# aliabdelkader/FusionTransformer

Measured on AMD Instinct MI355X. Metric: frames/sec fwd+bwd (SemanticKITTI synth), whole job, higher is better.
Workload: dtype f32

## Files before the change

fusiontransformer_amd/_lib.py:

```python
from __future__ import annotations

import ctypes as C
import os

import torch

_HERE = os.path.dirname(os.path.abspath(__file__))
LIB_PATH = os.path.join(_HERE, "csrc", "libftx.so")

_i32, _i64, _f32, _vp, _sz = C.c_int32, C.c_int64, C.c_float, C.c_void_p, C.c_size_t

SIGNATURES = {
    "ftx_version": (C.c_int, []),
    "ftx_last_error": (C.c_char_p, []),
    "ftx_stream_scratch_bytes": (_sz, []),
    "ftx_stream_scratch_attach": (C.c_int, [_vp, _vp, _sz]),
    "ftx_stream_scratch_reset": (C.c_int, [_vp]),
    "ftx_stream_scratch_release": (C.c_int, [_vp]),
    "ftx_hash": (C.c_int, [_vp, _i64, _vp, _vp]),
    "ftx_hash_kernel": (C.c_int, [_vp, _i64, _vp, _i32, _vp, _vp]),
    "ftx_floor_coords": (C.c_int, [_vp, _i64, _i32, _vp, _vp]),
    "ftx_hashtable_capacity": (_i64, [_i64]),
    "ftx_hashtable_build": (C.c_int, [_vp, _i64, _vp, _vp, _i64, _vp]),
    "ftx_hashtable_query": (C.c_int, [_vp, _i64, _vp, _vp, _i64, _vp, _vp]),
# ... 37 lines not shown
    "ftx_spconv_ostat": (C.c_int, [_vp, _i64, _vp, _i64, _vp, _i32, _i32, _i32, _i32, _i32, _vp, _vp, _i32, _vp]),
    "ftx_rows_gemm": (C.c_int, [_vp, _i64, _vp, _i32, _vp, _i32, _i32, _vp, _vp]),
    "ftx_spconv_gemm_block_cols": (_i32, [_i32, _i64, _i32]),
    "ftx_spconv_reduce": (C.c_int, [_vp, _vp, _i64, _i32, _i32, _vp, _vp]),
    "ftx_spconv_reduce_bn_eval": (C.c_int, [_vp, _vp, _i64, _i32, _i32, _vp, _vp, _vp, _vp, _vp, _f32, _i32, _vp, _vp]),
    "ftx_spconv_reduce_stats_blocks": (_i32, [_i64, _i32]),
    "ftx_spconv_reduce_stats": (C.c_int, [_vp, _vp, _i64, _i32, _i32, _vp, _vp, _i32, _vp]),
    "ftx_bn_train_fwd_totals": (C.c_int, [_vp, _vp, _vp, _vp, _vp, _vp, _f32, _f32, _i64, _i32, _i32, _vp, _vp, _vp, _vp, _vp]),
    "ftx_spconv_pairs_wgrad_workspace_bytes": (_sz, [_i64, _i32, _i32, _i32]),
    "ftx_spconv_pairs_wgrad": (C.c_int, [_vp, _i64, _vp, _vp, _i64, _vp, _vp, _i64, _i32, _i32, _i32, _vp, _vp, _sz, _vp]),
    "ftx_spconv_wgrad_resident_blocks": (_i32, [_i32, _i32]),
    "ftx_spconv_wgrad_table_blocks": (_i32, [_i32, _i32, _i32, _i32]),
    "ftx_spconv_pairs_gemm_bf16": (C.c_int, [_vp, _i64, _vp, _vp, _i32, _vp, _i64, _i32, _i32, _i32, _vp, _vp]),
    "ftx_spconv_pairs_gemm_scatter_bf16": (C.c_int, [_vp, _i64, _vp, _vp, _vp, _i32, _vp, _i64, _i32, _i32, _i32, _vp, _i64, _vp]),
    "ftx_rows_gemm_bf16": (C.c_int, [_vp, _i64, _vp, _i32, _vp, _i32, _i32, _vp, _vp]),
    "ftx_spconv_pairs_wgrad_bf16_workspace_bytes": (_sz, [_i64, _i32, _i32, _i32]),
    "ftx_spconv_pairs_wgrad_bf16": (C.c_int, [_vp, _i64, _vp, _vp, _i64, _vp, _vp, _i64, _i32, _i32, _i32, _vp, _vp, _sz, _vp]),
    "ftx_spconv_gemm_bf16_block_cols": (_i32, [_i32, _i64, _i32]),
    "ftx_spconv_wgrad_bf16_table_blocks": (_i32, [_i32, _i32, _i32, _i32]),
    "ftx_bn_workspace_bytes": (_sz, [_i64, _i32]),
    "ftx_bn_train_fwd": (C.c_int, [_vp, _vp, _vp, _vp, _vp, _vp, _f32, _f32, _i64, _i32, _i32, _vp, _vp, _vp, _vp, _sz, _vp]),
    "ftx_bn_eval_fwd": (C.c_int, [_vp, _vp, _vp, _vp, _vp, _vp, _f32, _i64, _i32, _i32, _vp, _vp]),
    "ftx_adam_chunk_elements": (_i32, []),
    "ftx_adam_tensor_bytes": (_i32, []),
    "ftx_adam_step": (C.c_int, [_vp, _vp, _vp, _i32, C.c_double, C.c_double, _f32, _f32, _vp]),
    "ftx_add_layernorm_fwd": (C.c_int, [_vp, _vp, _vp, _vp, _vp, _f32, _i64, _i32, _vp, _vp, _vp, _vp, _vp]),
    "ftx_layernorm_bwd_workspace_bytes": (_sz, [_i64, _i32]),
    "ftx_add_layernorm_bwd": (C.c_int, [_vp, _vp, _vp, _vp, _vp, _vp, _i64, _i32, _i32, _vp, _vp, _vp, _sz, _vp]),
    "ftx_colsum_workspace_bytes": (_sz, [_i64, _i32]),
    "ftx_colsum": (C.c_int, [_vp, _i64, _i32, _vp, _vp, _sz, _vp]),
    "ftx_attn_fwd": (C.c_int, [_vp, _i32, _i32, _i32, _i32, _f32, _vp, _vp, _vp]),
    "ftx_attn_bwd_workspace_bytes": (_sz, [_i32, _i32, _i32]),
    "ftx_attn_bwd": (C.c_int, [_vp, _vp, _vp, _vp, _i32, _i32, _i32, _i32, _f32, _vp, _vp, _sz, _vp]),
    "ftx_attn_fwd_tiled": (C.c_int, [_vp, _i32, _i32, _i32, _i32, _f32, _vp, _vp, _i32, _i32, _vp]),
    "ftx_attn_bwd_tiled": (C.c_int, [_vp, _vp, _vp, _vp, _i32, _i32, _i32, _i32, _f32, _vp, _vp, _sz, _i32, _i32, _vp]),
    "ftx_attn_fwd_bf16": (C.c_int, [_vp, _i32, _i32, _i32, _i32, _f32, _vp, _vp, _i32, _i32, _vp]),
    "ftx_attn_bwd_bf16": (C.c_int, [_vp, _vp, _vp, _vp, _i32, _i32, _i32, _i32, _f32, _vp, _vp, _sz, _i32, _i32, _vp]),
    "ftx_dense_gemm_bf16": (C.c_int, [_vp, _vp, _i32, _vp, _vp, _i64, _i32, _i32, _i32, _vp, _vp, _vp]),
    "ftx_dense_wgrad_bf16_workspace_bytes": (_sz, [_i64, _i32, _i32]),
    "ftx_dense_wgrad_bf16": (C.c_int, [_vp, _vp, _i64, _i32, _i32, _vp, _vp, _sz, _vp]),
    "ftx_dense_bf16_tile": (C.c_int, [_i32, _i64, _i32, _i32, _vp, _vp, _vp]),
    "ftx_dense_gemm_split": (C.c_int, [_vp, _vp, _i32, _vp, _vp, _i64, _i32, _i32, _i32, _vp, _vp, _vp]),
    "ftx_dense_wgrad_split_workspace_bytes": (_sz, [_i64, _i32, _i32]),
    "ftx_dense_wgrad_split": (C.c_int, [_vp, _vp, _i64, _i32, _i32, _vp, _vp, _sz, _vp]),
    "ftx_dense_split_tile": (C.c_int, [_i32, _i64, _i32, _i32, _vp, _vp, _vp]),
    "ftx_fusion_loss_workspace_bytes": (_sz, []),
    "ftx_fusion_loss": (C.c_int, [_vp, _vp, _vp, _vp, _vp, _vp, _f32, _i64, _i32, _i32, _vp, _vp, _vp, _vp, _vp, _vp, _vp, _vp, _sz, _vp]),
    "ftx_fusion_loss_mix": (C.c_int, [_vp, _vp, _vp, _vp, _vp, _vp, _f32, _f32, _i64, _i32, _i32, _vp, _vp, _vp, _vp, _vp, _vp, _vp, _vp, _sz, _vp]),
    "ftx_seg_loss_workspace_bytes": (_sz, []),
    "ftx_seg_loss": (C.c_int, [_vp, _vp, _vp, _i64, _i32, _i32, _vp, _vp, _vp, _vp, _sz, _vp]),
    "ftx_project_points": (C.c_int, [_vp, _i64, _vp, _i32, _i32, _vp, _vp, _vp]),
    "ftx_eval_scatter_back": (C.c_int, [_vp, _vp, _i64, _i32, _vp, _vp, _i64, _vp, _vp, _vp, _vp, _vp, _vp, _vp, _vp, _vp]),
    "ftx_bn_train_bwd": (C.c_int, [_vp, _vp, _vp, _vp, _vp, _vp, _vp, _i64, _i32, _i32, _vp, _vp, _vp, _vp, _vp, _sz, _vp]),
    "ftx_color_jitter_workspace_bytes": (_sz, [_i32, _i32]),
    "ftx_color_jitter_u8": (C.c_int, [_vp, _i64, _i32, _i32, _i32, _vp, _vp, _i32, _vp, _vp, _sz, _vp]),
    "ftx_color_jitter_chw": (C.c_int, [_vp, _i64, _i32, _i32, _i32, _vp, _vp, _i32, _i32, _vp, _vp, _vp, _vp, _sz, _vp]),
    "ftx_resize_ksize": (_i32, [_i32, _i32]),
    "ftx_resize_coeffs_host": (C.c_int, [_i32, _i32, _vp, _vp]),
    "ftx_resize_workspace_bytes": (_sz, [_i32, _i32, _i32, _i32, _i32]),
    "ftx_resize_bilinear_u8": (C.c_int, [_vp, _i64, _i64, _i32, _i32, _i32, _i32, _vp, _vp, _i32, _vp, _vp, _i32, _i32, _i32, _vp, _vp, _sz, _vp]),
    "ftx_rows_concat": (C.c_int, [_vp, _i32, _vp, _i32, _i64, _vp, _vp]),
    "ftx_rows_add": (C.c_int, [_vp, _vp, _i64, _i32, _vp, _vp]),
    "ftx_spvcnn_layer_bytes": (_i32, []),
    "ftx_spvcnn_op_bytes": (_i32, []),
    "ftx_spvcnn_map_bytes": (_i32, []),
    "ftx_spvcnn_pv_bytes": (_i32, []),
# ... 64 lines not shown
```

fusiontransformer_amd/csrc/ftx_attn.hip:

```cpp
#include "ftx_common.h"
#include "ftx_mfma.h"

using namespace ftx;

constexpr int HD = 64;
constexpr int TS = 68;
constexpr float LOG2E = 1.4426950408889634f;
constexpr float LN2 = 0.6931471805599453f;

__device__ inline int acc_row(int g, int h) { return (g & 3) + 8 * (g >> 2) + 4 * h; }

__device__ inline float exp2_raw(float x) { return __builtin_amdgcn_exp2f(x); }

__device__ inline const float *qkv_row(const float *qkv, int b, int t, int which, int hd, int T, int nh) {
  return qkv + ((((int64_t)b * T + t) * 3 + which) * nh + hd) * HD;
}

__device__ inline void load_frag(const float *row, int h, bool valid, float (&f)[32]) {
#pragma unroll
  for (int t = 0; t < 8; ++t) {
    float4 v = make_float4(0.f, 0.f, 0.f, 0.f);
    if (valid) v = *(const float4 *)(row + 8 * t + 4 * h);
    f[4 * t + 0] = v.x; f[4 * t + 1] = v.y; f[4 * t + 2] = v.z; f[4 * t + 3] = v.w;
  }
// ... 209 lines not shown
    const float inv = 1.f / l;
    float *op = out + (((int64_t)b * T + q) * nh + hd) * HD;
#pragma unroll
    for (int g4 = 0; g4 < 4; ++g4) {
      int r = acc_row(4 * g4, h);
      *(float4 *)(op + r) = make_float4(o0[4 * g4] * inv, o0[4 * g4 + 1] * inv, o0[4 * g4 + 2] * inv, o0[4 * g4 + 3] * inv);
      *(float4 *)(op + 32 + r) = make_float4(o1[4 * g4] * inv, o1[4 * g4 + 1] * inv, o1[4 * g4 + 2] * inv, o1[4 * g4 + 3] * inv);
    }
    if (h == 0) lse[((int64_t)b * nh + hd) * T + q] = (m + log2f(l)) * LN2;
  }
}

__global__ void attn_delta_kernel(const float *__restrict__ o, const float *__restrict__ go, int64_t rows, int T, int nh, float *__restrict__ delta) {
  const int64_t gid = (blockIdx.x * (int64_t)blockDim.x + threadIdx.x) >> 4;
  const int sub = threadIdx.x & 15;
  if (gid >= rows) return;
  float4 a = *(const float4 *)(o + gid * HD + sub * 4);
  float4 g = *(const float4 *)(go + gid * HD + sub * 4);
  float s = a.x * g.x + a.y * g.y + a.z * g.z + a.w * g.w;
#pragma unroll
  for (int off = 8; off > 0; off >>= 1) s += __shfl_xor(s, off, 16);
  if (sub == 0) {
    int64_t bt = gid / nh;
    int hd = (int)(gid - bt * nh);
    int64_t bb = bt / T;
    int t = (int)(bt - bb * T);
    delta[(bb * nh + hd) * T + t] = s;
  }
}

template <int QW, int SPLIT>
__global__ __launch_bounds__(64 * QW * SPLIT) void attn_bwd_kv_kernel(const float *__restrict__ qkv, const float *__restrict__ go,
                                                                      const float *__restrict__ lse, const float *__restrict__ delta, int T,
                                                                      int nh, float scale, float *__restrict__ gqkv) {
  constexpr int NT = 64 * QW;
  __shared__ __attribute__((aligned(16))) float smem[smem_floats<QW, SPLIT, 64, 64>()];
  const int tid = threadIdx.x % NT, grp = threadIdx.x / NT;
  float *Qs = smem + grp * (2 * 32 * TS + 64), *Gs = Qs + 32 * TS, *s_lse = Gs + 32 * TS, *s_delta = s_lse + 32;
  const int wave = tid >> 6, lane = tid & 63, l31 = lane & 31, h = lane >> 5;
  const int hd = blockIdx.y, b = blockIdx.z;
  const int key = blockIdx.x * (32 * QW) + wave * 32 + l31;
  const bool kv = key < T;
  const bool wave_live = blockIdx.x * (32 * QW) + wave * 32 < T;
  const float sl2 = scale * LOG2E;

  float kf[32], vf[32];
  load_frag(qkv_row(qkv, b, kv ? key : 0, 1, hd, T, nh), h, kv, kf);
  load_frag(qkv_row(qkv, b, kv ? key : 0, 2, hd, T, nh), h, kv, vf);
#pragma unroll
  for (int i = 0; i < 32; ++i) kf[i] *= sl2;

  f32x16 acc[4];
#pragma unroll
  for (int t = 0; t < 4; ++t)
#pragma unroll
    for (int g = 0; g < 16; ++g) acc[t][g] = 0.f;

  const int ntiles = (T + 31) / 32;
  const int iters = (ntiles + SPLIT - 1) / SPLIT;
  float4 rq[512 / NT], rg[512 / NT];
  tile_prefetch<NT>(qkv, b, hd, 0, grp * 32, T, nh, tid, rq);
  tile_prefetch_o<NT>(go, b, hd, grp * 32, T, nh, tid, rg);
  for (int it = 0; it < iters; ++it) {
    const int qt = it * SPLIT + grp;
    tile_store<NT>(Qs, tid, rq);
    tile_store<NT>(Gs, tid, rg);
    if (tid < 32) {
      int t = qt * 32 + tid;
      s_lse[tid] = t < T ? lse[((int64_t)b * nh + hd) * T + t] * LOG2E : 0.f;
      s_delta[tid] = t < T ? delta[((int64_t)b * nh + hd) * T + t] : 0.f;
    }
    group_sync<QW>();
    if (it + 1 < iters) {
      tile_prefetch<NT>(qkv, b, hd, 0, (qt + SPLIT) * 32, T, nh, tid, rq);
      tile_prefetch_o<NT>(go, b, hd, (qt + SPLIT) * 32, T, nh, tid, rg);
    }
    if (qt < ntiles && wave_live) {
      f32x16 s, dp;
#pragma unroll
      for (int g = 0; g < 16; ++g) s[g] = dp[g] = 0.f;
      mfma_lds_x_frag(Qs, l31, h, kf, s);
      mfma_lds_x_frag(Gs, l31, h, vf, dp);
#pragma unroll
      for (int g = 0; g < 16; ++g) {
        const int r = acc_row(g, h);
        const float p = exp2_raw(s[g] - s_lse[r]);
        s[g] = p;
        dp[g] = p * (dp[g] - s_delta[r]) * scale;
      }
      if (qt == ntiles - 1) {
#pragma unroll
        for (int g = 0; g < 16; ++g)
          if (qt * 32 + acc_row(g, h) >= T) s[g] = dp[g] = 0.f;
      }
      mfma_ldsT_x_acc(Gs, 0, l31, h, s, acc[0]);
      mfma_ldsT_x_acc(Gs, 32, l31, h, s, acc[1]);
      mfma_ldsT_x_acc(Qs, 0, l31, h, dp, acc[2]);
      mfma_ldsT_x_acc(Qs, 32, l31, h, dp, acc[3]);
    }
    group_sync<QW>();
  }
  merge_sum<QW, SPLIT, 4>(smem, grp, wave, lane, acc);
  if (kv && grp == 0) {
    float *kp = gqkv + ((((int64_t)b * T + key) * 3 + 1) * nh + hd) * HD;
    float *vp = gqkv + ((((int64_t)b * T + key) * 3 + 2) * nh + hd) * HD;
#pragma unroll
    for (int g4 = 0; g4 < 4; ++g4) {
      int r = acc_row(4 * g4, h);
      *(float4 *)(vp + r) = make_float4(acc[0][4 * g4], acc[0][4 * g4 + 1], acc[0][4 * g4 + 2], acc[0][4 * g4 + 3]);
      *(float4 *)(vp + 32 + r) = make_float4(acc[1][4 * g4], acc[1][4 * g4 + 1], acc[1][4 * g4 + 2], acc[1][4 * g4 + 3]);
      *(float4 *)(kp + r) = make_float4(acc[2][4 * g4], acc[2][4 * g4 + 1], acc[2][4 * g4 + 2], acc[2][4 * g4 + 3]);
      *(float4 *)(kp + 32 + r) = make_float4(acc[3][4 * g4], acc[3][4 * g4 + 1], acc[3][4 * g4 + 2], acc[3][4 * g4 + 3]);
    }
  }
}

template <int QW, int SPLIT>
__global__ __launch_bounds__(64 * QW * SPLIT) void attn_bwd_q_kernel(const float *__restrict__ qkv, const float *__restrict__ go,
                                                                     const float *__restrict__ lse, const float *__restrict__ delta, int T,
                                                                     int nh, float scale, float *__restrict__ gqkv) {
  constexpr int NT = 64 * QW;
  __shared__ __attribute__((aligned(16))) float smem[smem_floats<QW, SPLIT, 32, 0>()];
  const int tid = threadIdx.x % NT, grp = threadIdx.x / NT;
  float *Ks = smem + grp * (2 * 32 * TS), *Vs = Ks + 32 * TS;
  const int wave = tid >> 6, lane = tid & 63, l31 = lane & 31, h = lane >> 5;
  const int hd = blockIdx.y, b = blockIdx.z;
// ... 31 lines not shown
    if (kt < ntiles && wave_live) {
      f32x16 st, dpt;
#pragma unroll
      for (int g = 0; g < 16; ++g) st[g] = dpt[g] = 0.f;
      mfma_lds_x_frag(Ks, l31, h, qf, st);
      mfma_lds_x_frag(Vs, l31, h, gf, dpt);
#pragma unroll
      for (int g = 0; g < 16; ++g) {
        const float p = exp2_raw(st[g] - my_lse);
        dpt[g] = p * (dpt[g] - my_delta) * scale;
      }
      if (kt == ntiles - 1) {
#pragma unroll
        for (int g = 0; g < 16; ++g)
          if (kt * 32 + acc_row(g, h) >= T) dpt[g] = 0.f;
      }
      mfma_ldsT_x_acc(Ks, 0, l31, h, dpt, acc[0]);
      mfma_ldsT_x_acc(Ks, 32, l31, h, dpt, acc[1]);
    }
    group_sync<QW>();
  }
  merge_sum<QW, SPLIT, 2>(smem, grp, wave, lane, acc);
  if (qv && grp == 0) {
    float *qp = gqkv + ((((int64_t)b * T + q) * 3 + 0) * nh + hd) * HD;
#pragma unroll
    for (int g4 = 0; g4 < 4; ++g4) {
      int r = acc_row(4 * g4, h);
      *(float4 *)(qp + r) = make_float4(acc[0][4 * g4], acc[0][4 * g4 + 1], acc[0][4 * g4 + 2], acc[0][4 * g4 + 3]);
      *(float4 *)(qp + 32 + r) = make_float4(acc[1][4 * g4], acc[1][4 * g4 + 1], acc[1][4 * g4 + 2], acc[1][4 * g4 + 3]);
    }
  }
}

static int attn_check(const char *who, int b, int t, int h, int d) {
  FTX_REQUIRE(b >= 1 && t >= 1 && h >= 1, "%s: bad size", who);
  FTX_REQUIRE(d == HD, "%s: head dim must be 64 (got %d)", who, d);
  FTX_REQUIRE(b <= 65535 && h <= 65535, "%s: batch / heads exceed the grid limits", who);
  return FTX_OK;
}

static bool attn_tiling_built(int qw, int split) {
  return (qw == 0 && split == 0) || (qw == 4 && split == 2) || (qw == 2 && (split == 2 || split == 4)) ||
         (qw == 1 && (split == 2 || split == 4 || split == 8));
}
static void attn_config(int b, int t, int h, bool backward, int &qw, int &split) {
  if (qw != 0) return;
  const int64_t wave_tiles = (int64_t)ceil_div(t, 32) * h * b;
  const int64_t simds = 4 * 256;
  if (wave_tiles * 4 <= simds) { qw = 1; split = backward ? 4 : 8; }
  else if (wave_tiles * 2 <= simds) { qw = 2; split = 4; }
  else { qw = 4; split = 2; }
}

#define ATTN_DISPATCH(KERNEL, ...)                                                                               \
  do {                                                                                                           \
    dim3 grid((unsigned)ceil_div(t, 32 * qw), (unsigned)h, (unsigned)b);                                         \
    if (qw == 4) KERNEL<4, 2><<<grid, 512, 0, st>>>(__VA_ARGS__);                                                \
    else if (qw == 2 && split == 2) KERNEL<2, 2><<<grid, 256, 0, st>>>(__VA_ARGS__);                             \
    else if (qw == 2) KERNEL<2, 4><<<grid, 512, 0, st>>>(__VA_ARGS__);                                           \
    else if (split == 2) KERNEL<1, 2><<<grid, 128, 0, st>>>(__VA_ARGS__);                                        \
    else if (split == 4) KERNEL<1, 4><<<grid, 256, 0, st>>>(__VA_ARGS__);                                        \
    else KERNEL<1, 8><<<grid, 512, 0, st>>>(__VA_ARGS__);                                                        \
  } while (0)

extern "C" int ftx_attn_fwd_tiled(const float *qkv, int32_t b, int32_t t, int32_t h, int32_t d, float scale, float *out, float *lse, int32_t qw,
                                  int32_t split, void *stream) {
  int rc = attn_check("ftx_attn_fwd", b, t, h, d);
  if (rc != FTX_OK) return rc;
  FTX_REQUIRE(qkv && out && lse, "ftx_attn_fwd: null pointer");
  FTX_REQUIRE(attn_tiling_built(qw, split), "ftx_attn_fwd_tiled: (%d, %d) is not a built tiling", qw, split);
  hipStream_t st = (hipStream_t)stream;
  attn_config(b, t, h, false, qw, split);
  ATTN_DISPATCH(attn_fwd_kernel, qkv, t, h, scale, out, lse);
  return check_launch("ftx_attn_fwd");
}

extern "C" int ftx_attn_fwd(const float *qkv, int32_t b, int32_t t, int32_t h, int32_t d, float scale, float *out, float *lse, void *stream) {
  return ftx_attn_fwd_tiled(qkv, b, t, h, d, scale, out, lse, 0, 0, stream);
}

extern "C" size_t ftx_attn_bwd_workspace_bytes(int32_t b, int32_t t, int32_t h) {
  if (b <= 0 || t <= 0 || h <= 0) return 256;
  return sizeof(float) * (size_t)b * t * h + 256;
}

extern "C" int ftx_attn_bwd_tiled(const float *qkv, const float *out, const float *grad_out, const float *lse, int32_t b, int32_t t, int32_t h,
                                  int32_t d, float scale, float *grad_qkv, void *workspace, size_t workspace_bytes, int32_t qw, int32_t split,
                                  void *stream) {
  int rc = attn_check("ftx_attn_bwd", b, t, h, d);
  if (rc != FTX_OK) return rc;
  FTX_REQUIRE(qkv && out && grad_out && lse && grad_qkv && workspace, "ftx_attn_bwd: null pointer");
  FTX_REQUIRE(attn_tiling_built(qw, split), "ftx_attn_bwd_tiled: (%d, %d) is not a built tiling", qw, split);
  if (workspace_bytes < ftx_attn_bwd_workspace_bytes(b, t, h)) {
    set_error("ftx_attn_bwd: workspace %zu < required %zu", workspace_bytes, ftx_attn_bwd_workspace_bytes(b, t, h));
    return FTX_EWORKSPACE;
  }
  hipStream_t st = (hipStream_t)stream;
  float *delta = (float *)workspace;
  const int64_t rows = (int64_t)b * t * h;
  attn_delta_kernel<<<(unsigned)ceil_div(rows * 16, 256), 256, 0, st>>>(out, grad_out, rows, t, h, delta);
  attn_config(b, t, h, true, qw, split);
  ATTN_DISPATCH(attn_bwd_kv_kernel, qkv, grad_out, lse, delta, t, h, scale, grad_qkv);
  ATTN_DISPATCH(attn_bwd_q_kernel, qkv, grad_out, lse, delta, t, h, scale, grad_qkv);
  return check_launch("ftx_attn_bwd");
}

extern "C" int ftx_attn_bwd(const float *qkv, const float *out, const float *grad_out, const float *lse, int32_t b, int32_t t, int32_t h,
                            int32_t d, float scale, float *grad_qkv, void *workspace, size_t workspace_bytes, void *stream) {
  return ftx_attn_bwd_tiled(qkv, out, grad_out, lse, b, t, h, d, scale, grad_qkv, workspace, workspace_bytes, 0, 0, stream);
}

constexpr int RS = 72;
constexpr int CS = 36;
constexpr int IMG = 32 * RS;
static_assert(32 * RS == 64 * CS, "row and col images are the same size");

__device__ inline bf16x4 cvt4(float4 v) { return (bf16x4){(__bf16)v.x, (__bf16)v.y, (__bf16)v.z, (__bf16)v.w}; }

__device__ inline void load_frag_bf16(const float *row, int h, bool valid, bf16x8 (&f)[4]) {
#pragma unroll
  for (int s = 0; s < 4; ++s) {
    float4 a = make_float4(0.f, 0.f, 0.f, 0.f), b = a;
    if (valid) {
      a = *(const float4 *)(row + 16 * s + 8 * h);
      b = *(const float4 *)(row + 16 * s + 8 * h + 4);
    }
    f[s] = __builtin_shufflevector(cvt4(a), cvt4(b), 0, 1, 2, 3, 4, 5, 6, 7);
  }
}
__device__ inline bf16x8 rowimg_frag(const __bf16 *img, int row, int s, int h) { return *(const bf16x8 *)(img + row * RS + 16 * s + 8 * h); }
__device__ inline bf16x8 colimg_frag(const __bf16 *img, int row, int s, int h) {
  const __bf16 *p = img + row * CS + 16 * s + 4 * h;
  return __builtin_shufflevector(*(const bf16x4 *)p, *(const bf16x4 *)(p + 8), 0, 1, 2, 3, 4, 5, 6, 7);
}
__device__ inline bf16x8 acc_frag(const f32x16 &x, int s) {
  bf16x8 r;
#pragma unroll
// ... 386 lines not shown
```

fusiontransformer_amd/csrc/ftx_index.hip:

```cpp
#include <cstring>
#include <cstdlib>
#include "ftx_common.h"
#include <rocprim/device/device_radix_sort.hpp>
#include <rocprim/device/device_select.hpp>
#include <string>

namespace ftx {
static thread_local std::string g_err;
void set_error(const char *fmt, ...) {
  char buf[512];
  va_list ap;
  va_start(ap, fmt);
  vsnprintf(buf, sizeof(buf), fmt, ap);
  va_end(ap);
  g_err = buf;
}
}

using namespace ftx;

extern "C" int ftx_version(void) { return 101; }
extern "C" const char *ftx_last_error(void) { return ftx::g_err.c_str(); }

__global__ void hash_kernel(const int4 *__restrict__ coords, int64_t n, int64_t *__restrict__ out) {
  for (int64_t i = blockIdx.x * (int64_t)blockDim.x + threadIdx.x; i < n; i += (int64_t)gridDim.x * blockDim.x) {
    int4 c = coords[i];
    out[i] = fnv_hash4(c.x, c.y, c.z, c.w);
  }
}

extern "C" int ftx_hash(const int32_t *coords, int64_t n, int64_t *out, void *stream) {
  FTX_REQUIRE(n >= 0, "ftx_hash: n < 0");
  if (n == 0) return FTX_OK;
  FTX_REQUIRE(coords && out, "ftx_hash: null pointer");
  hash_kernel<<<grid_for(n, 256), 256, 0, (hipStream_t)stream>>>((const int4 *)coords, n, out);
  return check_launch("ftx_hash");
}

__global__ void hash_kernel_offsets(const int4 *__restrict__ coords, int64_t n, const int32_t *__restrict__ offsets, int k,
                                    int64_t *__restrict__ out) {
  int64_t total = n * k;
  for (int64_t e = blockIdx.x * (int64_t)blockDim.x + threadIdx.x; e < total; e += (int64_t)gridDim.x * blockDim.x) {
    int kk = (int)(e / n);
    int64_t i = e - (int64_t)kk * n;
    int4 c = coords[i];
    out[e] = fnv_hash4(c.x + offsets[kk * 3 + 0], c.y + offsets[kk * 3 + 1], c.z + offsets[kk * 3 + 2], c.w);
  }
}

extern "C" int ftx_hash_kernel(const int32_t *coords, int64_t n, const int32_t *offsets, int32_t k, int64_t *out, void *stream) {
  FTX_REQUIRE(n >= 0 && k >= 0, "ftx_hash_kernel: negative size");
  if (n == 0 || k == 0) return FTX_OK;
  FTX_REQUIRE(coords && offsets && out, "ftx_hash_kernel: null pointer");
  hash_kernel_offsets<<<grid_for(n * k, 256), 256, 0, (hipStream_t)stream>>>((const int4 *)coords, n, offsets, k, out);
// ... 483 lines not shown
```

fusiontransformer_amd/functional.py:

```python
from __future__ import annotations

import ctypes
import functools

import numpy as np
import torch

from . import _lib
from ._lib import check, ptr, req, stream

I32, I64, F32 = torch.int32, torch.int64, torch.float32


def _empty(shape, dtype, like):
    return torch.empty(shape, dtype=dtype, device=like.device)


_SCRATCH = {}
_WS_BYTES = {}


def _ws_bytes(fn_name, *args):
    key = (fn_name,) + args
    v = _WS_BYTES.get(key)
# ... 1052 lines not shown
            g = gs if gs is not None else torch.zeros(ctx.shape, dtype=F32, device=s.device)
            gyb = colsum(g.reshape(-1, g.shape[-1])) if ctx.with_y_bias else None
            return g, g, gyb, None, None, None
        gx, gparams = _ln_backward(gh, gs, s, weight, stats, ctx.with_y_bias)
        gx = gx.view(ctx.shape)
        return gx, gx, (gparams[2] if ctx.with_y_bias else None), gparams[0], gparams[1], None


def layer_norm(x, weight, bias, eps=1e-5):
    return _LayerNorm.apply(x, weight, bias, eps)


def add_layer_norm(x, y, weight, bias, eps=1e-5, y_bias=None):
    return _AddLayerNorm.apply(x, y, y_bias, weight, bias, eps)


def colsum(x: torch.Tensor) -> torch.Tensor:
    L = _lib.load()
    x = req(x.contiguous(), F32, "colsum x", 2)
    rows, cols = x.shape
    out = _empty((cols,), F32, x)
    ws_bytes = _ws_bytes("ftx_colsum_workspace_bytes", rows, cols)
    ws = _scratch(ws_bytes, x)
    check(L.ftx_colsum(ptr(x), rows, cols, ptr(out), ptr(ws), ws_bytes, stream()), "ftx_colsum")
    return out


_ATTENTION = {False: ("ftx_attn_fwd_tiled", "attn_fwd", "ftx_attn_bwd_tiled", "attn_bwd"),
              True: ("ftx_attn_fwd_bf16", "attn_fwd_bf16", "ftx_attn_bwd_bf16", "attn_bwd_bf16")}


class _Attention(torch.autograd.Function):
    @staticmethod
    def forward(ctx, qkv, scale, tiling=(0, 0), bf16=False):
        L = _lib.load()
        fn, kind = _ATTENTION[bf16][:2]
        qkv = req(qkv.contiguous(), F32, "attention qkv", 5)
        b, t, three, h, d = qkv.shape
        if three != 3 or d != 64:
            raise ValueError(f"attention: qkv must be (B, T, 3, heads, 64), got {tuple(qkv.shape)}")
        out = _empty((b, t, h * d), F32, qkv)
        lse = _empty((b, h, t), F32, qkv)
        qw, split = int(tiling[0]), int(tiling[1])
        _log_launch(kind, dict(b=b, t=t, h=h, d=d, products=2), lambda: check(getattr(L, fn)(
            ptr(qkv), b, t, h, d, float(scale), ptr(out), ptr(lse), qw, split, stream()), fn))
        ctx.save_for_backward(qkv, out, lse)
        ctx.scale, ctx.tiling, ctx.bf16 = float(scale), (qw, split), bf16
        return out

    @staticmethod
    def backward(ctx, go):
        L = _lib.load()
        fn, kind = _ATTENTION[ctx.bf16][2:]
        qkv, out, lse = ctx.saved_tensors
        b, t, _, h, d = qkv.shape
        go = req(go.contiguous(), F32, "attention grad", 3)
        gqkv = torch.empty_like(qkv)
        ws_bytes = int(L.ftx_attn_bwd_workspace_bytes(b, t, h))
        ws = torch.empty((ws_bytes,), dtype=torch.uint8, device=qkv.device)
        _log_launch(kind, dict(b=b, t=t, h=h, d=d, products=7), lambda: check(getattr(L, fn)(
            ptr(qkv), ptr(out), ptr(go), ptr(lse), b, t, h, d, ctx.scale, ptr(gqkv), ptr(ws), ws_bytes, ctx.tiling[0], ctx.tiling[1], stream()), fn))
        return gqkv, None, None, None


def attention(qkv, scale, tiling=(0, 0), bf16=False):
    return _Attention.apply(qkv, scale, tiling, bool(bf16))


EPI_NONE, EPI_BIAS, EPI_BIAS_GELU, EPI_DGELU = 0, 1, 2, 3
_DENSE_MODES = ("bf16", "split")


def vit_linear_supported(x, weight):
    n, k = weight.shape
    return (x.is_cuda and weight.is_cuda and x.dtype == F32 and weight.dtype == F32 and x.shape[-1] == k and k % 64 == 0 and n % 64 == 0
            and x.numel() // k <= (1 << 30))


def _dense_gemm(a, w, w_kn, epi, bias=None, pre_in=None, with_pre=False, mode="bf16"):
    L = _lib.load()
    m, kr = a.shape
    n = w.shape[1] if w_kn else w.shape[0]
    out = _empty((m, n), F32, a)
    pre = _empty((m, n), F32, a) if with_pre else None
    _log_launch("vit_gemm_" + mode, dict(m=m, n=n, k=kr, w_kn=w_kn, epi=epi), lambda: check(getattr(L, "ftx_dense_gemm_" + mode)(
        ptr(a), ptr(w), w_kn, ptr(bias), ptr(pre_in), m, n, kr, epi, ptr(out), ptr(pre), stream()), "ftx_dense_gemm_" + mode))
    return out, pre


def _dense_wgrad(g, x, mode="bf16"):
    L = _lib.load()
    m, n = g.shape
    k = x.shape[1]
    dw = _empty((n, k), F32, g)
    ws_bytes = _ws_bytes(f"ftx_dense_wgrad_{mode}_workspace_bytes", m, n, k)
    ws = _scratch(ws_bytes, g)
    _log_launch("vit_wgrad_" + mode, dict(m=m, n=n, k=k), lambda: check(getattr(L, "ftx_dense_wgrad_" + mode)(
        ptr(g), ptr(x), m, n, k, ptr(dw), ptr(ws), ws_bytes, stream()), "ftx_dense_wgrad_" + mode))
    return dw
# ... 381 lines not shown
```

include/ftx.h:

```cpp
#ifndef FTX_H
#define FTX_H

#include <stddef.h>
#include <stdint.h>

#ifdef __cplusplus
extern "C" {
#endif

#define FTX_OK 0
#define FTX_EINVAL -1
#define FTX_ELAUNCH -2
#define FTX_EWORKSPACE -3

int ftx_version(void);
const char *ftx_last_error(void);

size_t ftx_stream_scratch_bytes(void);
int ftx_stream_scratch_attach(void *stream, void *buffer, size_t bytes);
int ftx_stream_scratch_reset(void *stream);
int ftx_stream_scratch_release(void *stream);


int ftx_hash(const int32_t *coords, int64_t n, int64_t *out, void *stream);
// ... 83 lines not shown
int32_t ftx_spconv_wgrad_table_blocks(int32_t mi, int32_t wmg, int32_t ni, int32_t wng);

int ftx_spconv_pairs_gemm_bf16(const float *A, int64_t rows_a, const int32_t *gather, const float *W, int32_t w_transposed, const int32_t *koff, int64_t n_pairs, int32_t ca, int32_t co, int32_t kvol, float *tmp, void *stream);
int ftx_spconv_pairs_gemm_scatter_bf16(const float *A, int64_t rows_a, const int32_t *gather, const int32_t *scatter, const float *W, int32_t w_transposed, const int32_t *koff, int64_t n_pairs, int32_t ca, int32_t co, int32_t kvol, float *out, int64_t rows_out, void *stream);
int ftx_rows_gemm_bf16(const float *A, int64_t n, const float *W, int32_t w_transposed, const float *bias, int32_t ca, int32_t co, float *out, void *stream);
size_t ftx_spconv_pairs_wgrad_bf16_workspace_bytes(int64_t n_pairs, int32_t ca, int32_t cg, int32_t kvol);
int ftx_spconv_pairs_wgrad_bf16(const float *A, int64_t rows_a, const int32_t *idx_a, const float *G, int64_t rows_g, const int32_t *idx_g, const int32_t *koff, int64_t n_pairs, int32_t ca, int32_t cg, int32_t kvol, float *dW, void *workspace, size_t workspace_bytes, void *stream);
int32_t ftx_spconv_gemm_bf16_block_cols(int32_t co, int64_t n_pairs, int32_t kvol);
int32_t ftx_spconv_wgrad_bf16_table_blocks(int32_t mi, int32_t wmg, int32_t ni, int32_t wng);


size_t ftx_bn_workspace_bytes(int64_t n, int32_t c);
int ftx_bn_train_fwd(const float *x, const float *residual, const float *gamma, const float *beta, float *running_mean, float *running_var, float momentum, float eps, int64_t n, int32_t c, int32_t relu, float *y, float *save_mean, float *save_invstd, void *workspace, size_t workspace_bytes, void *stream);
int ftx_bn_train_fwd_totals(const float *x, const float *residual, const float *gamma, const float *beta, float *running_mean, float *running_var, float momentum, float eps, int64_t n, int32_t c, int32_t relu, float *y, float *save_mean, float *save_invstd, const double *totals, void *stream);

int ftx_bn_eval_fwd(const float *x, const float *residual, const float *gamma, const float *beta, const float *running_mean, const float *running_var, float eps, int64_t n, int32_t c, int32_t relu, float *y, void *stream);
int ftx_bn_train_bwd(const float *grad_y, const float *x, const float *y, const float *gamma, const float *beta, const float *save_mean, const float *save_invstd, int64_t n, int32_t c, int32_t relu, float *grad_x, float *grad_residual, float *grad_gamma, float *grad_beta, void *workspace, size_t workspace_bytes, void *stream);

int32_t ftx_adam_chunk_elements(void);
int32_t ftx_adam_tensor_bytes(void);
int ftx_adam_step(const void *table, const int32_t *chunk_tensor, const int64_t *chunk_offset, int32_t n_chunks, double beta1, double beta2, float eps, float weight_decay, void *stream);

int ftx_add_layernorm_fwd(const float *x, const float *y, const float *y_bias, const float *gamma, const float *beta, float eps, int64_t rows, int32_t c, float *s_out, float *h_out, float *mean, float *rstd, void *stream);
size_t ftx_layernorm_bwd_workspace_bytes(int64_t rows, int32_t c);
int ftx_add_layernorm_bwd(const float *grad_h, const float *grad_s, const float *s, const float *gamma, const float *mean, const float *rstd, int64_t rows, int32_t c, int32_t with_y_bias, float *grad_x, float *grad_params, void *workspace, size_t workspace_bytes, void *stream);

size_t ftx_colsum_workspace_bytes(int64_t rows, int32_t cols);
int ftx_colsum(const float *x, int64_t rows, int32_t cols, float *out, void *workspace, size_t workspace_bytes, void *stream);


int ftx_attn_fwd(const float *qkv, int32_t b, int32_t t, int32_t h, int32_t d, float scale, float *out, float *lse, void *stream);
size_t ftx_attn_bwd_workspace_bytes(int32_t b, int32_t t, int32_t h);
int ftx_attn_bwd(const float *qkv, const float *out, const float *grad_out, const float *lse, int32_t b, int32_t t, int32_t h, int32_t d, float scale, float *grad_qkv, void *workspace, size_t workspace_bytes, void *stream);
int ftx_attn_fwd_tiled(const float *qkv, int32_t b, int32_t t, int32_t h, int32_t d, float scale, float *out, float *lse, int32_t qw, int32_t split, void *stream);
int ftx_attn_bwd_tiled(const float *qkv, const float *out, const float *grad_out, const float *lse, int32_t b, int32_t t, int32_t h, int32_t d, float scale, float *grad_qkv, void *workspace, size_t workspace_bytes, int32_t qw, int32_t split, void *stream);
int ftx_attn_fwd_bf16(const float *qkv, int32_t b, int32_t t, int32_t h, int32_t d, float scale, float *out, float *lse, int32_t qw, int32_t split, void *stream);
int ftx_attn_bwd_bf16(const float *qkv, const float *out, const float *grad_out, const float *lse, int32_t b, int32_t t, int32_t h, int32_t d, float scale, float *grad_qkv, void *workspace, size_t workspace_bytes, int32_t qw, int32_t split, void *stream);

#define FTX_EPI_NONE 0
#define FTX_EPI_BIAS 1
#define FTX_EPI_BIAS_GELU 2
#define FTX_EPI_DGELU 3
int ftx_dense_gemm_bf16(const float *A, const float *W, int32_t w_kn, const float *bias, const float *pre_in, int64_t m, int32_t n, int32_t k, int32_t epilogue, float *out, float *pre_out, void *stream);
size_t ftx_dense_wgrad_bf16_workspace_bytes(int64_t m, int32_t n, int32_t k);
int ftx_dense_wgrad_bf16(const float *dY, const float *X, int64_t m, int32_t n, int32_t k, float *dW, void *workspace, size_t workspace_bytes, void *stream);
int ftx_dense_bf16_tile(int32_t form, int64_t m, int32_t n, int32_t k, int32_t *tile_m_host, int32_t *tile_n_host, int32_t *split_host);

int ftx_dense_gemm_split(const float *A, const float *W, int32_t w_kn, const float *bias, const float *pre_in, int64_t m, int32_t n, int32_t k, int32_t epilogue, float *out, float *pre_out, void *stream);
size_t ftx_dense_wgrad_split_workspace_bytes(int64_t m, int32_t n, int32_t k);
int ftx_dense_wgrad_split(const float *dY, const float *X, int64_t m, int32_t n, int32_t k, float *dW, void *workspace, size_t workspace_bytes, void *stream);
int ftx_dense_split_tile(int32_t form, int64_t m, int32_t n, int32_t k, int32_t *tile_m_host, int32_t *tile_n_host, int32_t *split_host);

size_t ftx_fusion_loss_workspace_bytes(void);
int ftx_fusion_loss_mix(const float *lidar_logit, const float *img_logit, const float *lidar_logit2, const float *img_logit2, const int64_t *label, const float *class_weights, float ce_scale, float lambda_xm, int64_t n, int32_t c, int32_t ignore_index, float *losses, float *grad_lidar, float *grad_img, float *grad_lidar2, float *grad_img2, int64_t *conf3d, int64_t *conf2d, void *workspace, size_t workspace_bytes, void *stream);
int ftx_fusion_loss(const float *lidar_logit, const float *img_logit, const float *lidar_logit2, const float *img_logit2, const int64_t *label, const float *class_weights, float lambda_xm, int64_t n, int32_t c, int32_t ignore_index, float *losses, float *grad_lidar, float *grad_img, float *grad_lidar2, float *grad_img2, int64_t *conf3d, int64_t *conf2d, void *workspace, size_t workspace_bytes, void *stream);

size_t ftx_seg_loss_workspace_bytes(void);
int ftx_seg_loss(const float *logit, const int64_t *label, const float *class_weights, int64_t n, int32_t c, int32_t ignore_index, float *loss, float *grad, int64_t *conf, void *workspace, size_t workspace_bytes, void *stream);

int ftx_eval_scatter_back(const float *logits3d, const float *logits2d, int64_t n_rows, int32_t num_classes, const int64_t *inverse, const int32_t *gt, int64_t m, const int32_t *class_labels, int32_t *pred3d, int32_t *pred2d, int32_t *pred_ens, int64_t *conf3d, int64_t *conf2d, int64_t *conf_ens, int32_t *bad_flag, void *stream);

int ftx_project_points(const float *points, int64_t n, const float *proj_matrix, int32_t width, int32_t height, uint8_t *keep, float *rowcol, void *stream);

#define FTX_JITTER_BRIGHTNESS 0
#define FTX_JITTER_CONTRAST 1
#define FTX_JITTER_SATURATION 2
// ... 57 lines not shown
```

Before: 149.3.

## Hand off dS from KV backward kernel to Q backward instead of recomputing

The KV backward kernel now writes the score gradient dS tile to a workspace buffer. A new Q-gradient kernel reads dS and K and multiplies them, so it no longer recomputes QK^T, the exponentials and dO·V^T. The hand-off path is chosen automatically when the dS buffer fits in 256 MB. This trades recompute FLOPs for an extra T×T-sized global write and read plus a larger workspace.

```diff
diff --git a/fusiontransformer_amd/_lib.py b/fusiontransformer_amd/_lib.py
--- a/fusiontransformer_amd/_lib.py
+++ b/fusiontransformer_amd/_lib.py
@@ -93,6 +93,8 @@
     "ftx_attn_fwd": (C.c_int, [_vp, _i32, _i32, _i32, _i32, _f32, _vp, _vp, _vp]),
     "ftx_attn_bwd_workspace_bytes": (_sz, [_i32, _i32, _i32]),
     "ftx_attn_bwd": (C.c_int, [_vp, _vp, _vp, _vp, _i32, _i32, _i32, _i32, _f32, _vp, _vp, _sz, _vp]),
+    "ftx_attn_bwd_mode_workspace_bytes": (_sz, [_i32, _i32, _i32, _i32]),
+    "ftx_attn_bwd_mode": (C.c_int, [_vp, _vp, _vp, _vp, _i32, _i32, _i32, _i32, _f32, _vp, _vp, _sz, _i32, _i32, _i32, _vp]),
     "ftx_attn_fwd_tiled": (C.c_int, [_vp, _i32, _i32, _i32, _i32, _f32, _vp, _vp, _i32, _i32, _vp]),
     "ftx_attn_bwd_tiled": (C.c_int, [_vp, _vp, _vp, _vp, _i32, _i32, _i32, _i32, _f32, _vp, _vp, _sz, _i32, _i32, _vp]),
     "ftx_attn_fwd_bf16": (C.c_int, [_vp, _i32, _i32, _i32, _i32, _f32, _vp, _vp, _i32, _i32, _vp]),
diff --git a/fusiontransformer_amd/csrc/ftx_attn.hip b/fusiontransformer_amd/csrc/ftx_attn.hip
--- a/fusiontransformer_amd/csrc/ftx_attn.hip
+++ b/fusiontransformer_amd/csrc/ftx_attn.hip
@@ -265,7 +265,7 @@
 template <int QW, int SPLIT>
 __global__ __launch_bounds__(64 * QW * SPLIT) void attn_bwd_kv_kernel(const float *__restrict__ qkv, const float *__restrict__ go,
                                                                       const float *__restrict__ lse, const float *__restrict__ delta, int T,
-                                                                      int nh, float scale, float *__restrict__ gqkv) {
+                                                                      int nh, float scale, float *__restrict__ gqkv, float *__restrict__ ds) {
   constexpr int NT = 64 * QW;
   __shared__ __attribute__((aligned(16))) float smem[smem_floats<QW, SPLIT, 64, 64>()];
   const int tid = threadIdx.x % NT, grp = threadIdx.x / NT;
@@ -325,6 +325,19 @@
 #pragma unroll
         for (int g = 0; g < 16; ++g)
           if (qt * 32 + acc_row(g, h) >= T) s[g] = dp[g] = 0.f;
+      }
+      if (ds) {
+        const int TP = 32 * ntiles;
+        float *tile = ds + (((int64_t)b * nh + hd) * T + __builtin_amdgcn_readfirstlane(qt) * 32) * TP;
+        const unsigned lane_off = 4 * h * TP + key;
+        if (qt == ntiles - 1) {
+#pragma unroll
+          for (int g = 0; g < 16; ++g)
+            if (qt * 32 + acc_row(g, h) < T) (tile + acc_row(g, 0) * TP)[lane_off] = kv ? dp[g] : 0.f;
+        } else {
+#pragma unroll
+          for (int g = 0; g < 16; ++g) (tile + acc_row(g, 0) * TP)[lane_off] = kv ? dp[g] : 0.f;
+        }
       }
       mfma_ldsT_x_acc(Gs, 0, l31, h, s, acc[0]);
       mfma_ldsT_x_acc(Gs, 32, l31, h, s, acc[1]);
@@ -422,6 +435,68 @@
   }
 }
 
+__device__ inline void ds_prefetch(const float *dsrow, int kt, bool valid, float4 (&r)[4]) {
+#pragma unroll
+  for (int j = 0; j < 4; ++j) {
+    float4 v = make_float4(0.f, 0.f, 0.f, 0.f);
+    if (valid) v = *(const float4 *)(dsrow + kt * 32 + 8 * j);
+    r[j] = v;
+  }
+}
+template <int QW, int SPLIT>
+__global__ __launch_bounds__(64 * QW * SPLIT) void attn_bwd_q_handoff_kernel(const float *__restrict__ qkv, const float *__restrict__ ds, int T,
+                                                                             int nh, float *__restrict__ gqkv) {
+  constexpr int NT = 64 * QW;
+  __shared__ __attribute__((aligned(16))) float smem[cmax(SPLIT * 32 * TS, cmax(SPLIT / 2, 1) * QW * 32 * 64)];
+  const int tid = threadIdx.x % NT, grp = threadIdx.x / NT;
+  float *Ks = smem + grp * (32 * TS);
+  const int wave = tid >> 6, lane = tid & 63, l31 = lane & 31, h = lane >> 5;
+  const int hd = blockIdx.y, b = blockIdx.z;
+  const int q = blockIdx.x * (32 * QW) + wave * 32 + l31;
+  const bool qv = q < T;
+  const bool wave_live = blockIdx.x * (32 * QW) + wave * 32 < T;
+
+  f32x16 acc[2];
+#pragma unroll
+  for (int g = 0; g < 16; ++g) acc[0][g] = acc[1][g] = 0.f;
+
+  const int ntiles = (T + 31) / 32;
+  const int iters = (ntiles + SPLIT - 1) / SPLIT;
+  const float *dsrow = ds + (((int64_t)b * nh + hd) * T + (qv ? q : 0)) * (32 * ntiles) + 4 * h;
+  float4 rk[512 / NT], rd[4];
+  tile_prefetch<NT>(qkv, b, hd, 1, grp * 32, T, nh, tid, rk);
+  ds_prefetch(dsrow, grp, qv && grp < ntiles, rd);
+  for (int it = 0; it < iters; ++it) {
+    const int kt = it * SPLIT + grp;
+    tile_store<NT>(Ks, tid, rk);
+    f32x16 dst;
+#pragma unroll
+    for (int j = 0; j < 4; ++j) {
+      dst[4 * j + 0] = rd[j].x; dst[4 * j + 1] = rd[j].y; dst[4 * j + 2] = rd[j].z; dst[4 * j + 3] = rd[j].w;
+    }
+    group_sync<QW>();
+    if (it + 1 < iters) {
+      tile_prefetch<NT>(qkv, b, hd, 1, (kt + SPLIT) * 32, T, nh, tid, rk);
+      ds_prefetch(dsrow, kt + SPLIT, qv && kt + SPLIT < ntiles, rd);
+    }
+    if (kt < ntiles && wave_live) {
+      mfma_ldsT_x_acc(Ks, 0, l31, h, dst, acc[0]);
+      mfma_ldsT_x_acc(Ks, 32, l31, h, dst, acc[1]);
+    }
+    group_sync<QW>();
+  }
+  merge_sum<QW, SPLIT, 2>(smem, grp, wave, lane, acc);
+  if (qv && grp == 0) {
+    float *qp = gqkv + ((((int64_t)b * T + q) * 3 + 0) * nh + hd) * HD;
+#pragma unroll
+    for (int g4 = 0; g4 < 4; ++g4) {
+      int r = acc_row(4 * g4, h);
+      *(float4 *)(qp + r) = make_float4(acc[0][4 * g4], acc[0][4 * g4 + 1], acc[0][4 * g4 + 2], acc[0][4 * g4 + 3]);
+      *(float4 *)(qp + 32 + r) = make_float4(acc[1][4 * g4], acc[1][4 * g4 + 1], acc[1][4 * g4 + 2], acc[1][4 * g4 + 3]);
+    }
+  }
+}
+
 static int attn_check(const char *who, int b, int t, int h, int d) {
   FTX_REQUIRE(b >= 1 && t >= 1 && h >= 1, "%s: bad size", who);
   FTX_REQUIRE(d == HD, "%s: head dim must be 64 (got %d)", who, d);
@@ -469,30 +544,53 @@
   return ftx_attn_fwd_tiled(qkv, b, t, h, d, scale, out, lse, 0, 0, stream);
 }
 
+constexpr size_t ATTN_HANDOFF_CAP = (size_t)256 << 20;
+static size_t attn_delta_bytes(int b, int t, int h) { return (sizeof(float) * (size_t)b * t * h + 255) / 256 * 256; }
+static size_t attn_ds_bytes(int b, int t, int h) { return sizeof(float) * (size_t)b * h * t * (32 * (size_t)ceil_div(t, 32)); }
+static int attn_bwd_rule(int b, int t, int h) { return attn_ds_bytes(b, t, h) <= ATTN_HANDOFF_CAP ? 1 : 0; }
+
+extern "C" size_t ftx_attn_bwd_mode_workspace_bytes(int32_t b, int32_t t, int32_t h, int32_t mode) {
+  if (b <= 0 || t <= 0 || h <= 0) return 256;
+  if (mode != 1) return sizeof(float) * (size_t)b * t * h + 256;
+  return attn_delta_bytes(b, t, h) + attn_ds_bytes(b, t, h);
+}
+
 extern "C" size_t ftx_attn_bwd_workspace_bytes(int32_t b, int32_t t, int32_t h) {
   if (b <= 0 || t <= 0 || h <= 0) return 256;
-  return sizeof(float) * (size_t)b * t * h + 256;
-}
-
-extern "C" int ftx_attn_bwd_tiled(const float *qkv, const float *out, const float *grad_out, const float *lse, int32_t b, int32_t t, int32_t h,
-                                  int32_t d, float scale, float *grad_qkv, void *workspace, size_t workspace_bytes, int32_t qw, int32_t split,
-                                  void *stream) {
+  return ftx_attn_bwd_mode_workspace_bytes(b, t, h, attn_bwd_rule(b, t, h));
+}
+
+extern "C" int ftx_attn_bwd_mode(const float *qkv, const float *out, const float *grad_out, const float *lse, int32_t b, int32_t t, int32_t h,
+                                 int32_t d, float scale, float *grad_qkv, void *workspace, size_t workspace_bytes, int32_t qw, int32_t split,
+                                 int32_t mode, void *stream) {
   int rc = attn_check("ftx_attn_bwd", b, t, h, d);
   if (rc != FTX_OK) return rc;
   FTX_REQUIRE(qkv && out && grad_out && lse && grad_qkv && workspace, "ftx_attn_bwd: null pointer");
   FTX_REQUIRE(attn_tiling_built(qw, split), "ftx_attn_bwd_tiled: (%d, %d) is not a built tiling", qw, split);
-  if (workspace_bytes < ftx_attn_bwd_workspace_bytes(b, t, h)) {
-    set_error("ftx_attn_bwd: workspace %zu < required %zu", workspace_bytes, ftx_attn_bwd_workspace_bytes(b, t, h));
+  FTX_REQUIRE(mode == 0 || mode == 1, "ftx_attn_bwd_mode: mode must be 0 (recompute) or 1 (hand-off), got %d", mode);
+  FTX_REQUIRE(mode == 0 || ((uintptr_t)workspace & 15) == 0, "ftx_attn_bwd_mode: the hand-off workspace must be 16-byte aligned");
+  const size_t need = ftx_attn_bwd_mode_workspace_bytes(b, t, h, mode);
+  if (workspace_bytes < need) {
+    set_error("ftx_attn_bwd: workspace %zu < required %zu", workspace_bytes, need);
     return FTX_EWORKSPACE;
   }
   hipStream_t st = (hipStream_t)stream;
   float *delta = (float *)workspace;
+  float *ds = mode == 1 ? (float *)((char *)workspace + attn_delta_bytes(b, t, h)) : nullptr;
   const int64_t rows = (int64_t)b * t * h;
   attn_delta_kernel<<<(unsigned)ceil_div(rows * 16, 256), 256, 0, st>>>(out, grad_out, rows, t, h, delta);
   attn_config(b, t, h, true, qw, split);
-  ATTN_DISPATCH(attn_bwd_kv_kernel, qkv, grad_out, lse, delta, t, h, scale, grad_qkv);
-  ATTN_DISPATCH(attn_bwd_q_kernel, qkv, grad_out, lse, delta, t, h, scale, grad_qkv);
+  ATTN_DISPATCH(attn_bwd_kv_kernel, qkv, grad_out, lse, delta, t, h, scale, grad_qkv, ds);
+  if (mode == 1) ATTN_DISPATCH(attn_bwd_q_handoff_kernel, qkv, ds, t, h, grad_qkv);
+  else ATTN_DISPATCH(attn_bwd_q_kernel, qkv, grad_out, lse, delta, t, h, scale, grad_qkv);
   return check_launch("ftx_attn_bwd");
+}
+
+extern "C" int ftx_attn_bwd_tiled(const float *qkv, const float *out, const float *grad_out, const float *lse, int32_t b, int32_t t, int32_t h,
+                                  int32_t d, float scale, float *grad_qkv, void *workspace, size_t workspace_bytes, int32_t qw, int32_t split,
+                                  void *stream) {
+  const int mode = (b >= 1 && t >= 1 && h >= 1) ? attn_bwd_rule(b, t, h) : 0;
+  return ftx_attn_bwd_mode(qkv, out, grad_out, lse, b, t, h, d, scale, grad_qkv, workspace, workspace_bytes, qw, split, mode, stream);
 }
 
 extern "C" int ftx_attn_bwd(const float *qkv, const float *out, const float *grad_out, const float *lse, int32_t b, int32_t t, int32_t h,
diff --git a/fusiontransformer_amd/csrc/ftx_index.hip b/fusiontransformer_amd/csrc/ftx_index.hip
--- a/fusiontransformer_amd/csrc/ftx_index.hip
+++ b/fusiontransformer_amd/csrc/ftx_index.hip
@@ -19,7 +19,7 @@
 
 using namespace ftx;
 
-extern "C" int ftx_version(void) { return 101; }
+extern "C" int ftx_version(void) { return 102; }
 extern "C" const char *ftx_last_error(void) { return ftx::g_err.c_str(); }
 
 __global__ void hash_kernel(const int4 *__restrict__ coords, int64_t n, int64_t *__restrict__ out) {
diff --git a/fusiontransformer_amd/functional.py b/fusiontransformer_amd/functional.py
--- a/fusiontransformer_amd/functional.py
+++ b/fusiontransformer_amd/functional.py
@@ -1108,9 +1108,11 @@
 
 class _Attention(torch.autograd.Function):
     @staticmethod
-    def forward(ctx, qkv, scale, tiling=(0, 0), bf16=False):
+    def forward(ctx, qkv, scale, tiling=(0, 0), bf16=False, bwd_mode=None):
         L = _lib.load()
         fn, kind = _ATTENTION[bf16][:2]
+        if bwd_mode is not None and (bf16 or int(bwd_mode) not in (0, 1)):
+            raise ValueError("attention: bwd_mode is 0 (recompute) or 1 (hand-off) and belongs to the fp32 kernels")
         qkv = req(qkv.contiguous(), F32, "attention qkv", 5)
         b, t, three, h, d = qkv.shape
         if three != 3 or d != 64:
@@ -1122,6 +1124,7 @@
             ptr(qkv), b, t, h, d, float(scale), ptr(out), ptr(lse), qw, split, stream()), fn))
         ctx.save_for_backward(qkv, out, lse)
         ctx.scale, ctx.tiling, ctx.bf16 = float(scale), (qw, split), bf16
+        ctx.bwd_mode = None if bwd_mode is None else int(bwd_mode)
         return out
 
     @staticmethod
@@ -1132,15 +1135,22 @@
         b, t, _, h, d = qkv.shape
         go = req(go.contiguous(), F32, "attention grad", 3)
         gqkv = torch.empty_like(qkv)
-        ws_bytes = int(L.ftx_attn_bwd_workspace_bytes(b, t, h))
-        ws = torch.empty((ws_bytes,), dtype=torch.uint8, device=qkv.device)
-        _log_launch(kind, dict(b=b, t=t, h=h, d=d, products=7), lambda: check(getattr(L, fn)(
-            ptr(qkv), ptr(out), ptr(go), ptr(lse), b, t, h, d, ctx.scale, ptr(gqkv), ptr(ws), ws_bytes, ctx.tiling[0], ctx.tiling[1], stream()), fn))
-        return gqkv, None, None, None
-
-
-def attention(qkv, scale, tiling=(0, 0), bf16=False):
-    return _Attention.apply(qkv, scale, tiling, bool(bf16))
+        if ctx.bwd_mode is None:
+            ws_bytes = int(L.ftx_attn_bwd_workspace_bytes(b, t, h))
+            ws = torch.empty((ws_bytes,), dtype=torch.uint8, device=qkv.device)
+            _log_launch(kind, dict(b=b, t=t, h=h, d=d, products=7), lambda: check(getattr(L, fn)(
+                ptr(qkv), ptr(out), ptr(go), ptr(lse), b, t, h, d, ctx.scale, ptr(gqkv), ptr(ws), ws_bytes, ctx.tiling[0], ctx.tiling[1], stream()), fn))
+        else:
+            ws_bytes = int(L.ftx_attn_bwd_mode_workspace_bytes(b, t, h, ctx.bwd_mode))
+            ws = torch.empty((ws_bytes,), dtype=torch.uint8, device=qkv.device)
+            _log_launch(kind, dict(b=b, t=t, h=h, d=d, products=7), lambda: check(L.ftx_attn_bwd_mode(
+                ptr(qkv), ptr(out), ptr(go), ptr(lse), b, t, h, d, ctx.scale, ptr(gqkv), ptr(ws), ws_bytes, ctx.tiling[0], ctx.tiling[1],
+                ctx.bwd_mode, stream()), "ftx_attn_bwd_mode"))
+        return gqkv, None, None, None, None
+
+
+def attention(qkv, scale, tiling=(0, 0), bf16=False, bwd_mode=None):
+    return _Attention.apply(qkv, scale, tiling, bool(bf16), bwd_mode)
 
 
 EPI_NONE, EPI_BIAS, EPI_BIAS_GELU, EPI_DGELU = 0, 1, 2, 3
diff --git a/include/ftx.h b/include/ftx.h
--- a/include/ftx.h
+++ b/include/ftx.h
@@ -139,6 +139,8 @@
 int ftx_attn_fwd(const float *qkv, int32_t b, int32_t t, int32_t h, int32_t d, float scale, float *out, float *lse, void *stream);
 size_t ftx_attn_bwd_workspace_bytes(int32_t b, int32_t t, int32_t h);
 int ftx_attn_bwd(const float *qkv, const float *out, const float *grad_out, const float *lse, int32_t b, int32_t t, int32_t h, int32_t d, float scale, float *grad_qkv, void *workspace, size_t workspace_bytes, void *stream);
+size_t ftx_attn_bwd_mode_workspace_bytes(int32_t b, int32_t t, int32_t h, int32_t mode);
+int ftx_attn_bwd_mode(const float *qkv, const float *out, const float *grad_out, const float *lse, int32_t b, int32_t t, int32_t h, int32_t d, float scale, float *grad_qkv, void *workspace, size_t workspace_bytes, int32_t qw, int32_t split, int32_t mode, void *stream);
 int ftx_attn_fwd_tiled(const float *qkv, int32_t b, int32_t t, int32_t h, int32_t d, float scale, float *out, float *lse, int32_t qw, int32_t split, void *stream);
 int ftx_attn_bwd_tiled(const float *qkv, const float *out, const float *grad_out, const float *lse, int32_t b, int32_t t, int32_t h, int32_t d, float scale, float *grad_qkv, void *workspace, size_t workspace_bytes, int32_t qw, int32_t split, void *stream);
 int ftx_attn_fwd_bf16(const float *qkv, int32_t b, int32_t t, int32_t h, int32_t d, float scale, float *out, float *lse, int32_t qw, int32_t split, void *stream);
```

Result: no change. 150.8 (median of 5 runs) (+1.0%).
